# cnosdb/cnosdb

Hardware: AMD Instinct MI355X
Metric: decoded+filtered values/sec & HBM GB/s, TSBS devops scan, 1/2/4/8 GPU (higher is better)
Workload: dtype f64; 1 GPU; tsbs-devops-scan (BASELINE configs[1]: 10k series x 1M pts, reference-shaped 125k-row pages, delta-ts + Gorilla-f64 decode, ts-range filter 50%, fused 5-min max/sum/count); series_per_gpu=10000, fields=1, page_rows=125000, n_buckets=3334, raw_page_bytes_per_gpu=7320251367, sub_batches=2

## Files before the change

### cnosdb_amd/csrc/gs_engine.cpp

```cpp
#include <hip/hip_runtime.h>
#include "../../include/cnosdb_gs.h"
#include "gs_internal.h"

#pragma clang diagnostic ignored "-Wunused-value"

#include <cstdio>
#include <cstring>
#include <cstdlib>
#include <vector>
#include <algorithm>
#include <string>

static thread_local char g_err[512] = "";
static GsStatus fail(GsStatus s, const char *msg) {
    snprintf(g_err, sizeof(g_err), "%s", msg);
    return s;
}
extern "C" const char *gs_last_error(void) { return g_err; }

#define HIP_TRY(expr)                                                          \
    do {                                                                       \
        hipError_t _e = (expr);                                                \
        if (_e != hipSuccess) {                                                \
            snprintf(g_err, sizeof(g_err), "%s: %s", #expr,                    \
// ... 2313 lines not shown
    const int lane = threadIdx.x;
    int64_t carry = 0;
    for (int t = 0; t < nblocks; t += 64) {
        int i = t + lane;
        int64_t v = (i < nblocks) ? blocksums[i] : 0;
        int64_t x = v;
        for (int off = 1; off < 64; off <<= 1) {
            int64_t u = __shfl_up(x, off, 64);
            if (lane >= off) x += u;
        }
        if (i < nblocks) blocksums[i] = carry + x - v;
        carry += __shfl(x, 63, 64);
    }
    if (lane == 0) out[n] = carry;
}

__global__ void k_scan_add(int n, int64_t *__restrict__ out,
                           const int64_t *__restrict__ blocksums) {
    int chunk = SCAN_BLOCK * SCAN_ITEMS;
    for (int i = blockIdx.x * blockDim.x + threadIdx.x; i < n;
         i += gridDim.x * blockDim.x)
        out[i] += blocksums[i / chunk];
}

__global__ void k_build_sgroups_out(const int32_t *__restrict__ first,
                                    int nsg,
                                    const int64_t *__restrict__ out_off,
                                    DevGroup *__restrict__ sg) {
    for (int s = blockIdx.x * blockDim.x + threadIdx.x; s < nsg;
         s += gridDim.x * blockDim.x) {
        int64_t a = out_off[first[s]];
        int64_t b = out_off[first[s + 1]];
        sg[s].row_off = a;
        sg[s].nrows = int32_t(b - a);
        sg[s].pad = 0;
    }
}

__global__ void k_spans_rle(const uint8_t *__restrict__ blob,
                            const DevPage *__restrict__ pages, int npages,
                            int64_t lo, int64_t hi,
                            int64_t *__restrict__ sp_start,
                            int64_t *__restrict__ sp_cnt,
                            int64_t *__restrict__ g_t0sel,
                            int64_t *__restrict__ g_delta,
                            unsigned *__restrict__ err) {
    for (int p = blockIdx.x * blockDim.x + threadIdx.x; p < npages;
         p += gridDim.x * blockDim.x) {
        DevPage pg = pages[p];
        const uint8_t *s = blob + pg.data_off + 1;
        uint64_t scaler = 1;
        unsigned s10 = s[0] & 0x0f;
        for (unsigned k = 0; k < s10; k++) scaler *= 10;
        const uint8_t *q = s + 1;
        int64_t first = int64_t(dev_be64(q));
        uint64_t dv; uint32_t nr;
        dev_varint(q + 8, pg.data_len - 10, &dv, &nr);
        int64_t delta = int64_t(dv * scaler);
        int64_t n = pg.nrows;
        int64_t st, en;
        if (delta < 0) { atomicOr(err, DERR_NONMONO); st = en = 0; }
        else if (delta == 0) {
            bool in = first >= lo && first <= hi;
            st = 0; en = in ? n : 0;
        } else {
            __int128 d = delta;
            __int128 a = (__int128)lo - first;
            __int128 b = (__int128)hi - first;
            __int128 s0 = a <= 0 ? 0 : (a + d - 1) / d;
            __int128 e0 = b < 0 ? 0 : b / d + 1;
            if (s0 > n) s0 = n;
            if (e0 > n) e0 = n;
            st = int64_t(s0);
            en = int64_t(e0);
        }
        if (en < st) en = st;
        sp_start[pg.grp] = st;
        sp_cnt[pg.grp] = en - st;
        g_t0sel[pg.grp] = first + st * delta;
        g_delta[pg.grp] = delta;
    }
}

__global__ void k_rle_ts_filtered(const uint8_t *__restrict__ blob,
                                  const DevPage *__restrict__ pages,
                                  int npages,
                                  const int64_t *__restrict__ sp_start,
                                  const int64_t *__restrict__ sp_cnt,
                                  const int64_t *__restrict__ out_off,
                                  int64_t *__restrict__ out_ts) {
    for (int p = blockIdx.x; p < npages; p += gridDim.x) {
        DevPage pg = pages[p];
        const uint8_t *s = blob + pg.data_off + 1;
        uint64_t scaler = 1;
        unsigned s10 = s[0] & 0x0f;
        for (unsigned k = 0; k < s10; k++) scaler *= 10;
        const uint8_t *q = s + 1;
        int64_t first = int64_t(dev_be64(q));
        uint64_t dv; uint32_t nr;
        dev_varint(q + 8, pg.data_len - 10, &dv, &nr);
        int64_t delta = int64_t(dv * scaler);
        int64_t st = sp_start[pg.grp], cnt = sp_cnt[pg.grp];
        int64_t *o = out_ts + out_off[pg.grp];
        const uint64_t base = uint64_t(first) + uint64_t(st) * uint64_t(delta);
        const int64_t head = int64_t((uintptr_t(o) >> 3) & 1);
        if (head && threadIdx.x == 0 && cnt > 0) o[0] = int64_t(base);
        const int64_t n2 = (cnt - head) >> 1;
        longlong2 *op = (longlong2 *)(o + head);
        for (int64_t q2 = threadIdx.x; q2 < n2; q2 += blockDim.x) {
            const uint64_t r0 = uint64_t(head) + 2 * uint64_t(q2);
            longlong2 v;
            v.x = int64_t(base + r0 * uint64_t(delta));
            v.y = int64_t(base + (r0 + 1) * uint64_t(delta));
            op[q2] = v;
        }
        if (((cnt - head) & 1) && threadIdx.x == 0 && cnt > 0)
            o[cnt - 1] = int64_t(base + uint64_t(cnt - 1) * uint64_t(delta));
    }
}

__global__ void k_gor_active(const DevGorChunk *__restrict__ chunks,
                             int nchunks,
                             const int64_t *__restrict__ sp_start,
                             const int64_t *__restrict__ sp_cnt,
                             int *__restrict__ active,
                             int *__restrict__ n_active,
                             DevAggMeta *__restrict__ pieces) {
    const int lane = threadIdx.x & 63;
    for (int i = blockIdx.x * blockDim.x + threadIdx.x; i < nchunks;
         i += gridDim.x * blockDim.x) {
        uint32_t grp = chunks[i].grp;
        int64_t row0 = int64_t(chunks[i].row0);
        int64_t rend = row0 + int64_t(chunks[i].cnt);
        int64_t lo = sp_start[grp];
        int64_t hi = lo + sp_cnt[grp];
        bool act = row0 < hi && rend > lo;
        if (pieces && !act) {
            uint32_t slot = chunks[i].slot;
            if (slot != GOR_NO_SLOT)
                *(int4 *)(pieces + 2 * size_t(slot)) =
                    make_int4(AGG_NO_PIECE, 0, AGG_NO_PIECE, 0);
        }
        uint64_t m = __ballot(act);
        if (m) {
            int leader = __ffsll((unsigned long long)m) - 1;
            int base = 0;
            if (lane == leader) base = atomicAdd(n_active, __popcll(m));
            base = __shfl(base, leader);
            if (act)
                active[base + __popcll(m & ((1ull << lane) - 1))] = i;
        }
    }
}

struct GorAggArgs {
    const int32_t *grp_sg;
    const int64_t *g_t0sel;
    const int64_t *g_delta;
    int64_t t0, bucket_ns;
    int nbuckets;
    double *pmax, *psum;
    long long *pcnt;
    DevAggMeta *pc_meta;
    DevAggVal *pc_val;
};

#define GS_AGG_FUSED_MIN_ROWS 2

#define GOR_PARK_NB (1 << 30)
#define GOR_FK_END 0
#define GOR_FK_CLEAN 1
#define GOR_FK_OVER 2

template <bool AGG>
__global__ void k_gor_chunks_filtered(const uint8_t *__restrict__ blob,
                                      const DevGorChunk *__restrict__ chunks,
                                      const int *__restrict__ active,
                                      const int *__restrict__ n_active,
                                      const int64_t *__restrict__ sp_start,
                                      const int64_t *__restrict__ sp_cnt,
                                      const int64_t *__restrict__ out_off,
                                      double *__restrict__ out,
                                      unsigned *__restrict__ err,
                                      GorAggArgs ag) {
    __shared__ double ring[GS_GOR_BLOCK / 64][GS_RING][64 + 1];
    __shared__ uint64_t fdesc[GS_GOR_BLOCK / 64][64][2];
    const int lane = threadIdx.x & 63;
    const int wv = threadIdx.x >> 6;
    auto rslot = ring[wv];
    const int nact = *n_active;
    int stride = gridDim.x * blockDim.x;
    int base_id = blockIdx.x * blockDim.x + threadIdx.x;
    int rounds = (nact + stride - 1) / stride;
    for (int rd = 0; rd < rounds; rd++) {
        int ai = base_id + rd * stride;
        bool have = ai < nact;
        DevGorChunk ch = chunks[active[have ? ai : 0]];
        int32_t sel_lo = int32_t(sp_start[ch.grp]);
        int32_t sel_hi = int32_t(sel_lo + sp_cnt[ch.grp]);
        if (!have) { sel_lo = 0; sel_hi = 0; }
// ... 535 lines not shown
    __syncthreads();
    for (int p = blockIdx.x * blockDim.x + threadIdx.x; p < npages;
         p += gridDim.x * blockDim.x) {
        EncPageSpec ps = pages[p];
        uint8_t *pg = out + int64_t(p) * cap;
        uint32_t bl = uint32_t(ps.nrows + 7) / 8;
        uint8_t *bs = pg + 16;
        for (uint32_t b = 0; b < bl; b++) {
            uint8_t byte = 0;
            for (int k = 0; k < 8; k++) {
                int32_t r = int32_t(b) * 8 + k;
                if (r < ps.nrows && (!valid || valid[ps.row_off + r]))
                    byte |= uint8_t(1u << k);
            }
            bs[b] = byte;
        }
        uint8_t *data = pg + 16 + bl;
        int64_t dl;
        if (kind == 2) {
            dl = dev_enc_gorilla((const double *)vals, valid, ps.row_off,
                                 ps.nrows, data);
        } else {
            if (valid) {
                bool av = true;
                for (int32_t r = 0; r < ps.nrows; r++)
                    if (!valid[ps.row_off + r]) { av = false; break; }
                if (!av) { atomicOr(err, DERR_FORMAT); lens[p] = -3; continue; }
            }
            dl = dev_enc_int((const int64_t *)vals, ps.row_off, ps.nrows,
                             data, kind == 0);
        }
        if (dl < 0) {
            atomicOr(err, DERR_FORMAT);
            lens[p] = dl;
            continue;
        }
        uint32_t crc = 0xFFFFFFFFu;
        for (int64_t i = 0; i < dl; i++)
            crc = crct[(crc ^ data[i]) & 0xFF] ^ (crc >> 8);
        crc ^= 0xFFFFFFFFu;
        pg[0] = uint8_t(bl >> 24); pg[1] = uint8_t(bl >> 16);
        pg[2] = uint8_t(bl >> 8); pg[3] = uint8_t(bl);
        dev_put_be64(pg + 4, uint64_t(ps.nrows));
        pg[12] = uint8_t(crc >> 24); pg[13] = uint8_t(crc >> 16);
        pg[14] = uint8_t(crc >> 8); pg[15] = uint8_t(crc);
        lens[p] = 16 + int64_t(bl) + dl;
    }
}


struct GsCtx {
    int device;
    hipStream_t stream;
    unsigned *d_err;
};

static int grid_for(int work, int per_block) {
    int blocks = (work + per_block - 1) / per_block;
    if (blocks > 2048) blocks = 2048;
    if (blocks < 1) blocks = 1;
    return blocks;
}

struct SlotPages {
    uint8_t ctype;
    std::vector<DevPage> host[PC_NCLASS];
    DevPage *dev[PC_NCLASS] = {nullptr, nullptr, nullptr};
    int n[PC_NCLASS] = {0, 0, 0};
    std::vector<int64_t> str_scr;
    int64_t str_total = 0;
    int64_t *d_str_scr = nullptr;
    DevGorChunk *d_gor_chunks = nullptr;
    int n_gor_chunks = 0;
    int32_t *d_gor_chunk_base = nullptr;
    DevGorChunk *d_gorn_chunks = nullptr;
    int n_gorn_chunks = 0;
    int32_t *d_gorn_chunk_base = nullptr;
    std::vector<int32_t> gor_grp_cbase;
    int32_t *d_sg_chunk_first = nullptr;
    int max_sg_chunks = 0;
    bool agg_fused_ok = false;
};

struct GsGroupSet {
    GsCtx *ctx = nullptr;
    uint8_t *d_blob = nullptr;
    size_t blob_len = 0;
    int64_t total_rows = 0;
    size_t ngroups = 0;
    uint32_t ncols = 0;
    std::vector<int64_t> row_offsets;
    std::vector<SlotPages> slots;
    DevGroup *d_groups = nullptr;
    DevGroup *d_sgroups = nullptr;
    int nsgroups = 0;
    std::vector<int32_t> sgroup_span;
    std::vector<int64_t> sgroup_row_off;
    DevGroup *d_sgroups_out = nullptr;
    int32_t *d_sgroup_first = nullptr;
    int64_t *d_blocksums = nullptr;
    hipEvent_t sev[6];
    bool sev_init = false;
    bool pending = false;
    int64_t *d_sp_start = nullptr;
    int64_t *d_sp_cnt = nullptr;
    int64_t *d_out_off = nullptr;
    int64_t *d_g_t0sel = nullptr;
    int64_t *d_g_delta = nullptr;
    int max_span = 0;
    int *d_gor_active = nullptr;
    int *d_gor_nactive = nullptr;
    size_t gor_active_cap = 0;
    int32_t *d_grp_sgroup = nullptr;
    DevAggMeta *d_agg_meta = nullptr;
    DevAggVal *d_agg_val = nullptr;
    size_t agg_pieces_cap = 0;
    int64_t min_pos_delta = INT64_MAX;
    uint8_t *d_str_scratch = nullptr;
    size_t str_scratch_cap = 0;
    int64_t *d_str_sz = nullptr;
    int64_t *d_str_pos = nullptr;
    int64_t *d_str_bsums = nullptr;
    size_t str_bsums_cap = 0;
    GsTimeRange *d_ranges = nullptr;
    size_t ranges_cap = 0;
    uint8_t *d_valid = nullptr;
    uint8_t *d_mask = nullptr;
    int64_t *d_sel_cnt = nullptr;
    bool any_nulls_field = false;
    double *d_pmax = nullptr;
    double *d_psum = nullptr;
    long long *d_pcnt = nullptr;
    size_t partials_cap = 0;
};

extern "C" {

int gs_device_count(void) {
    int n = 0;
    if (hipGetDeviceCount(&n) != hipSuccess) return 0;
    return n;
}

GsCtx *gs_ctx_create(int device) {
    int n = 0;
    if (hipGetDeviceCount(&n) != hipSuccess || n == 0) {
        fail(GS_ERR_NO_GPU, "no HIP device available — cnosdb_gs has no CPU fallback");
        return nullptr;
    }
    if (device < 0 || device >= n) {
        fail(GS_ERR, "device index out of range");
        return nullptr;
    }
    HIP_TRY_NULL(hipSetDevice(device));
    GsCtx *ctx = new GsCtx();
    ctx->device = device;
    if (hipStreamCreate(&ctx->stream) != hipSuccess ||
        hipMalloc(&ctx->d_err, sizeof(unsigned)) != hipSuccess) {
        fail(GS_ERR, "ctx init failed");
        delete ctx;
        return nullptr;
    }
    hipMemset(ctx->d_err, 0, sizeof(unsigned));
    return ctx;
}

void gs_ctx_destroy(GsCtx *ctx) {
    if (!ctx) return;
    hipSetDevice(ctx->device);
    hipStreamSynchronize(ctx->stream);
    hipFree(ctx->d_err);
    hipStreamDestroy(ctx->stream);
    delete ctx;
}

GsGroupSet *gs_groups_upload(GsCtx *ctx, const GsColumnGroupDesc *groups,
                             size_t ngroups, int validate_crc) {
    if (!ctx || !groups || ngroups == 0) {
        fail(GS_ERR, "bad args to gs_groups_upload");
        return nullptr;
    }
    HIP_TRY_NULL(hipSetDevice(ctx->device));
    uint32_t ncols = groups[0].npages;
    for (size_t g = 0; g < ngroups; g++) {
// ... 391 lines not shown
        hipMalloc(&set->d_sgroup_first, sgfirst.size() * sizeof(int32_t)) != hipSuccess ||
        hipMalloc(&set->d_sgroups_out, hsg.size() * sizeof(DevGroup)) != hipSuccess ||
        hipMalloc(&set->d_g_t0sel, ngroups * sizeof(int64_t)) != hipSuccess ||
        hipMalloc(&set->d_g_delta, ngroups * sizeof(int64_t)) != hipSuccess) {
        fail(GS_ERR, "hipMalloc group tables failed");
        gs_groups_free(set); return nullptr;
    }
    for (int32_t sp : set->sgroup_span)
        if (sp > set->max_span) set->max_span = sp;
    hipMemcpyAsync(set->d_sgroup_first, sgfirst.data(),
                   sgfirst.size() * sizeof(int32_t), hipMemcpyHostToDevice,
                   ctx->stream);
    hipMemcpyAsync(set->d_groups, hg.data(), ngroups * sizeof(DevGroup),
                   hipMemcpyHostToDevice, ctx->stream);
    std::vector<int32_t> grp_sg(ngroups);
    for (size_t s = 0; s < hsg.size(); s++)
        for (int32_t g = sgfirst[s]; g < sgfirst[s + 1]; g++)
            grp_sg[g] = int32_t(s);
    std::vector<std::vector<int32_t>> sgc(ncols);
    if (hipMalloc(&set->d_grp_sgroup, ngroups * sizeof(int32_t)) != hipSuccess) {
        fail(GS_ERR, "hipMalloc group->sgroup table failed");
        gs_groups_free(set); return nullptr;
    }
    hipMemcpyAsync(set->d_grp_sgroup, grp_sg.data(),
                   ngroups * sizeof(int32_t), hipMemcpyHostToDevice,
                   ctx->stream);
    for (uint32_t c = 0; c < ncols; c++) {
        SlotPages &sp = set->slots[c];
        if (!sp.agg_fused_ok) continue;
        std::vector<int32_t> &t = sgc[c];
        t.resize(hsg.size() + 1);
        for (size_t s = 0; s <= hsg.size(); s++)
            t[s] = sp.gor_grp_cbase[sgfirst[s]];
        if (t[0] != 0 || t[hsg.size()] > sp.n_gor_chunks)
            sp.agg_fused_ok = false;
        for (size_t s = 0; s < hsg.size() && sp.agg_fused_ok; s++) {
            if (t[s + 1] < t[s]) sp.agg_fused_ok = false;
            if (t[s + 1] - t[s] > sp.max_sg_chunks)
                sp.max_sg_chunks = t[s + 1] - t[s];
        }
        if (!sp.agg_fused_ok) continue;
        if (hipMalloc(&sp.d_sg_chunk_first, t.size() * sizeof(int32_t)) != hipSuccess) {
            fail(GS_ERR, "hipMalloc sgroup chunk table failed");
            gs_groups_free(set); return nullptr;
        }
        hipMemcpyAsync(sp.d_sg_chunk_first, t.data(),
                       t.size() * sizeof(int32_t), hipMemcpyHostToDevice,
                       ctx->stream);
    }
    HIP_TRY_NULL(hipStreamSynchronize(ctx->stream));
    return set;
}

void gs_groups_free(GsGroupSet *set) {
    if (!set) return;
    hipSetDevice(set->ctx->device);
    hipStreamSynchronize(set->ctx->stream);
    for (auto &sp : set->slots) {
        for (int k = 0; k < PC_NCLASS; k++)
            if (sp.dev[k]) hipFree(sp.dev[k]);
        if (sp.d_str_scr) hipFree(sp.d_str_scr);
        if (sp.d_gor_chunks) hipFree(sp.d_gor_chunks);
        if (sp.d_gor_chunk_base) hipFree(sp.d_gor_chunk_base);
        if (sp.d_gorn_chunks) hipFree(sp.d_gorn_chunks);
        if (sp.d_gorn_chunk_base) hipFree(sp.d_gorn_chunk_base);
        if (sp.d_sg_chunk_first) hipFree(sp.d_sg_chunk_first);
    }
    if (set->d_grp_sgroup) hipFree(set->d_grp_sgroup);
    if (set->d_agg_meta) hipFree(set->d_agg_meta);
    if (set->d_agg_val) hipFree(set->d_agg_val);
    if (set->d_gor_active) hipFree(set->d_gor_active);
    if (set->d_gor_nactive) hipFree(set->d_gor_nactive);
    if (set->d_str_scratch) hipFree(set->d_str_scratch);
    if (set->d_str_sz) hipFree(set->d_str_sz);
    if (set->d_str_pos) hipFree(set->d_str_pos);
    if (set->d_str_bsums) hipFree(set->d_str_bsums);
    hipFree(set->d_blob);
    hipFree(set->d_groups);
    if (set->d_sgroups) hipFree(set->d_sgroups);
    if (set->d_sgroups_out) hipFree(set->d_sgroups_out);
    if (set->d_sgroup_first) hipFree(set->d_sgroup_first);
    if (set->d_blocksums) hipFree(set->d_blocksums);
    if (set->sev_init)
        for (int k = 0; k < 6; k++) hipEventDestroy(set->sev[k]);
    hipFree(set->d_sp_start);
    hipFree(set->d_sp_cnt);
    hipFree(set->d_out_off);
    if (set->d_g_t0sel) hipFree(set->d_g_t0sel);
    if (set->d_g_delta) hipFree(set->d_g_delta);
    if (set->d_ranges) hipFree(set->d_ranges);
    if (set->d_valid) hipFree(set->d_valid);
    if (set->d_mask) hipFree(set->d_mask);
    if (set->d_sel_cnt) hipFree(set->d_sel_cnt);
    if (set->d_pmax) hipFree(set->d_pmax);
    if (set->d_psum) hipFree(set->d_psum);
    if (set->d_pcnt) hipFree(set->d_pcnt);
    delete set;
}

int64_t gs_debug_gorn_table(GsCtx *ctx, GsGroupSet *set, uint32_t col,
                            DevGorChunk *out, int64_t cap) {
    if (!ctx || !set || col >= set->ncols) return -1;
    SlotPages &sp = set->slots[col];
    int64_t n = sp.n_gorn_chunks;
    if (!out || cap < n) return n;
    hipSetDevice(ctx->device);
    hipStreamSynchronize(ctx->stream);
    if (hipMemcpy(out, sp.d_gorn_chunks, size_t(n) * sizeof(DevGorChunk),
                  hipMemcpyDeviceToHost) != hipSuccess)
        return -1;
    return n;
}

int64_t gs_debug_read_blob(GsCtx *ctx, GsGroupSet *set, uint64_t off,
                           uint64_t len, uint8_t *out) {
    if (!ctx || !set || off + len > set->blob_len) return -1;
    hipSetDevice(ctx->device);
    hipStreamSynchronize(ctx->stream);
    if (hipMemcpy(out, set->d_blob + off, len, hipMemcpyDeviceToHost) !=
        hipSuccess)
        return -1;
    return int64_t(len);
}

int64_t gs_debug_rerun_gorn_sync(GsCtx *ctx, GsGroupSet *set,
                                 uint32_t col) {
    if (!ctx || !set || col >= set->ncols) return -1;
    SlotPages &sp = set->slots[col];
    if (!sp.n[PC_GORN]) return 0;
    hipSetDevice(ctx->device);
    const char *e = getenv("GS_GOR_CHUNK");
    long v = e ? atol(e) : 0;
    uint32_t chunk_rows = uint32_t(v >= 64 ? v : GOR_CHUNK);
    hipLaunchKernelGGL(k_gor_sync_null, dim3(grid_for(sp.n[PC_GORN], 256)),
                       dim3(256), 0, ctx->stream, set->d_blob,
                       sp.dev[PC_GORN], sp.n[PC_GORN], sp.d_gorn_chunk_base,
                       sp.d_gorn_chunks, chunk_rows);
    hipStreamSynchronize(ctx->stream);
    return 1;
}

__global__ void k_debug_crc(const uint8_t *__restrict__ p, uint64_t len,
                            uint64_t *__restrict__ out) {
    uint64_t acc = 0;
    for (uint64_t i = blockIdx.x * blockDim.x + threadIdx.x; i < len;
         i += uint64_t(gridDim.x) * blockDim.x)
        acc += (uint64_t(p[i]) + 1) * (i + 0x9e3779b97f4a7c15ULL);
    atomicAdd((unsigned long long *)out, (unsigned long long)acc);
}

int64_t gs_debug_kernel_crc(GsCtx *ctx, GsGroupSet *set, uint64_t off,
                            uint64_t len, uint64_t *out_sum) {
    if (!ctx || !set || off + len > set->blob_len) return -1;
    hipSetDevice(ctx->device);
    uint64_t *d;
    if (hipMalloc(&d, 8) != hipSuccess) return -1;
    hipMemset(d, 0, 8);
    hipLaunchKernelGGL(k_debug_crc, dim3(64), dim3(256), 0, ctx->stream,
                       set->d_blob + off, len, d);
    hipStreamSynchronize(ctx->stream);
    hipMemcpy(out_sum, d, 8, hipMemcpyDeviceToHost);
    hipFree(d);
    return 0;
}

int64_t gs_set_rows(const GsGroupSet *set) { return set ? set->total_rows : -1; }
int64_t gs_set_series(const GsGroupSet *set) { return set ? set->nsgroups : -1; }
// ... 317 lines not shown
                      (SCAN_BLOCK * SCAN_ITEMS));
    if (set->str_bsums_cap < size_t(nblocks) + 1) {
        if (set->d_str_bsums) hipFree(set->d_str_bsums);
        if (hipMalloc(&set->d_str_bsums, (size_t(nblocks) + 1) * 8) != hipSuccess)
            return fail(GS_ERR, "hipMalloc string scan sums failed");
        set->str_bsums_cap = size_t(nblocks) + 1;
    }
    hipLaunchKernelGGL(k_str_decode, dim3(grid_for(n, 256)), dim3(256), 0,
                       ctx->stream, set->d_blob, sp.dev[PC_STR], n,
                       sp.d_str_scr, set->d_str_scratch, set->d_str_sz,
                       set->d_str_pos, d_valid, ctx->d_err);
    hipLaunchKernelGGL(k_scan_partials, dim3(nblocks), dim3(SCAN_BLOCK), 0,
                       ctx->stream, set->d_str_sz, int(set->total_rows),
                       d_offsets, set->d_str_bsums);
    hipLaunchKernelGGL(k_scan_fixup, dim3(1), dim3(64), 0, ctx->stream,
                       int(set->total_rows), d_offsets, set->d_str_bsums,
                       nblocks);
    hipLaunchKernelGGL(k_scan_add, dim3(grid_for(int(set->total_rows), 256)),
                       dim3(256), 0, ctx->stream, int(set->total_rows),
                       d_offsets, set->d_str_bsums);
    int64_t total = 0;
    HIP_TRY(hipMemcpyAsync(&total, d_offsets + set->total_rows, 8,
                           hipMemcpyDeviceToHost, ctx->stream));
    HIP_TRY(hipStreamSynchronize(ctx->stream));
    GsStatus st = check_dev_err(ctx);
    if (st != GS_OK) return st;
    if (total > bytes_cap)
        return fail(GS_ERR, "string bytes buffer too small");
    hipLaunchKernelGGL(k_str_gather, dim3(grid_for(int(set->total_rows), 256)),
                       dim3(256), 0, ctx->stream, set->d_str_scratch,
                       set->d_str_pos, set->d_str_sz, d_offsets,
                       set->total_rows, d_bytes);
    HIP_TRY(hipStreamSynchronize(ctx->stream));
    *total_bytes = total;
    return check_dev_err(ctx);
}

GsStatus gs_apply_tombstone(GsCtx *ctx, GsGroupSet *set, const int64_t *d_ts,
                            uint8_t *d_valid, const GsTimeRange *ranges,
                            size_t nranges) {
    if (!ctx || !set || !d_ts || !d_valid || !ranges || nranges == 0)
        return fail(GS_ERR, "bad args to gs_apply_tombstone");
    HIP_TRY(hipSetDevice(ctx->device));
    if (set->ranges_cap < nranges) {
        if (set->d_ranges) hipFree(set->d_ranges);
        HIP_TRY(hipMalloc(&set->d_ranges, nranges * sizeof(GsTimeRange)));
        set->ranges_cap = nranges;
    }
    HIP_TRY(hipMemcpyAsync(set->d_ranges, ranges, nranges * sizeof(GsTimeRange),
                           hipMemcpyHostToDevice, ctx->stream));
    int blocks = int(set->ngroups > 2048 ? 2048 : set->ngroups);
    hipLaunchKernelGGL(k_tombstone, dim3(blocks), dim3(256), 0, ctx->stream,
                       set->d_groups, int(set->ngroups), d_ts, d_valid,
                       set->d_ranges, int(nranges));
    HIP_TRY(hipStreamSynchronize(ctx->stream));
    return GS_OK;
}

static bool fused_capable_fields(GsGroupSet *set, const GsScanSpec *spec,
                                 const int32_t *fields, int nf) {
    if (!(spec->d_out_ts && spec->d_out_val && spec->n_tombstones == 0 &&
          spec->value_pred.op == GS_PRED_NONE && !set->any_nulls_field &&
          set->slots[0].n[PC_RLE_TS] == int(set->ngroups)))
        return false;
    for (int f = 0; f < nf; f++) {
        uint32_t fc = 1 + uint32_t(fields[f]);
        if (fc >= set->ncols ||
            set->slots[fc].n[PC_GOR] != int(set->ngroups))
            return false;
    }
    return true;
}

static bool fused_capable(GsGroupSet *set, const GsScanSpec *spec) {
    int32_t f0 = spec->field_col;
    return fused_capable_fields(set, spec, &f0, 1);
}

static GsStatus scan_fused_launch(GsCtx *ctx, GsGroupSet *set,
                                  const GsScanSpec *spec,
                                  const int32_t *fields, int nf) {
    HIP_TRY(hipSetDevice(ctx->device));
    if (!set->sev_init) {
        for (int k = 0; k < 6; k++) HIP_TRY(hipEventCreate(&set->sev[k]));
        set->sev_init = true;
    }
    hipEvent_t *ev = set->sev;
    int ng = int(set->ngroups);
    const DevPage *ts_pages = set->slots[0].dev[PC_RLE_TS];
    int nch_max = 0;
    for (int f = 0; f < nf; f++) {
        int nc = set->slots[1 + fields[f]].n_gor_chunks;
        nch_max = nc > nch_max ? nc : nch_max;
    }
    if (!set->d_gor_nactive &&
        hipMalloc(&set->d_gor_nactive, sizeof(int)) != hipSuccess)
        return fail(GS_ERR, "hipMalloc active counter failed");
    if (set->gor_active_cap < size_t(nch_max)) {
        if (set->d_gor_active) hipFree(set->d_gor_active);
        if (hipMalloc(&set->d_gor_active, size_t(nch_max) * sizeof(int)) !=
            hipSuccess)
            return fail(GS_ERR, "hipMalloc active list failed");
        set->gor_active_cap = size_t(nch_max);
    }
    int nblocks = (ng + SCAN_BLOCK * SCAN_ITEMS - 1) /
                  (SCAN_BLOCK * SCAN_ITEMS);
    if (nblocks > 2048)
        return fail(GS_ERR, "too many groups for the fused span scan");
    HIP_TRY(hipEventRecord(ev[0], ctx->stream));
    hipLaunchKernelGGL(k_spans_rle, dim3(grid_for(ng, 256)), dim3(256), 0,
                       ctx->stream, set->d_blob, ts_pages, ng,
                       spec->range.min_ts, spec->range.max_ts,
                       set->d_sp_start, set->d_sp_cnt, set->d_g_t0sel,
                       set->d_g_delta, ctx->d_err);
    hipLaunchKernelGGL(k_scan_partials, dim3(nblocks), dim3(SCAN_BLOCK), 0,
                       ctx->stream, set->d_sp_cnt, ng, set->d_out_off,
                       set->d_blocksums);
    hipLaunchKernelGGL(k_scan_fixup, dim3(1), dim3(64), 0, ctx->stream, ng,
                       set->d_out_off, set->d_blocksums, nblocks);
    hipLaunchKernelGGL(k_scan_add, dim3(grid_for(ng, 256)), dim3(256), 0,
                       ctx->stream, ng, set->d_out_off, set->d_blocksums);
    HIP_TRY(hipEventRecord(ev[1], ctx->stream));
    hipLaunchKernelGGL(k_rle_ts_filtered, dim3(ng > 2048 ? 2048 : ng),
                       dim3(256), 0, ctx->stream, set->d_blob, ts_pages, ng,
                       set->d_sp_start, set->d_sp_cnt, set->d_out_off,
                       spec->d_out_ts);
    HIP_TRY(hipEventRecord(ev[2], ctx->stream));
    int nsg = set->nsgroups;
    if (spec->n_buckets > 0) {
        if (!spec->d_agg_max || !spec->d_agg_sum || !spec->d_agg_count)
            return fail(GS_ERR, "agg outputs missing");
        size_t cells = size_t(nsg) * size_t(spec->n_buckets);
        if (set->partials_cap < cells) {
            if (set->d_pmax) hipFree(set->d_pmax);
            if (set->d_psum) hipFree(set->d_psum);
            if (set->d_pcnt) hipFree(set->d_pcnt);
            if (hipMalloc(&set->d_pmax, cells * 8) != hipSuccess ||
                hipMalloc(&set->d_psum, cells * 8) != hipSuccess ||
                hipMalloc(&set->d_pcnt, cells * 8) != hipSuccess)
                return fail(GS_ERR, "hipMalloc agg partials failed");
            set->partials_cap = cells;
        }
    }
    bool sgroups_built = false;
    auto build_sgroups = [&]() {
        if (sgroups_built) return;
        hipLaunchKernelGGL(k_build_sgroups_out, dim3(grid_for(nsg, 256)),
                           dim3(256), 0, ctx->stream, set->d_sgroup_first,
                           nsg, set->d_out_off, set->d_sgroups_out);
        sgroups_built = true;
    };
    for (int f = 0; f < nf; f++) {
        SlotPages &fsp = set->slots[1 + fields[f]];
        int nch = fsp.n_gor_chunks;
        double *d_val_f = spec->d_out_val + size_t(f) * set->total_rows;
        HIP_TRY(hipMemsetAsync(set->d_gor_nactive, 0, sizeof(int),
                               ctx->stream));
        const size_t shm_rle =
            size_t(set->max_span) * 16 +
            (size_t(set->max_span) + size_t(spec->n_buckets) + 2) * 4;
        const bool rle_fits =
            spec->n_buckets <= 8192 && shm_rle <= 64 * 1024;
        const size_t shm_fix =
            (size_t(fsp.max_sg_chunks) * 2 * 4 + size_t(spec->n_buckets) +
             15) & ~size_t(15);
        bool agg_fused = false;
        if (spec->n_buckets > 0 && rle_fits && fsp.agg_fused_ok &&
            spec->bucket_ns > 0 && shm_fix <= 64 * 1024) {
            static int fused_env = [] {
                const char *e = getenv("GS_AGG_FUSED");
                return e ? atoi(e) : 1;
            }();
            static long min_rows = [] {
                const char *e = getenv("GS_AGG_FUSED_MIN_ROWS");
                long v = e ? atol(e) : 0;
                return v > 0 ? v : long(GS_AGG_FUSED_MIN_ROWS);
            }();
            agg_fused = fused_env != 0 &&
                        (set->min_pos_delta == INT64_MAX ||
                         spec->bucket_ns / set->min_pos_delta >= min_rows);
        }
        if (agg_fused && set->agg_pieces_cap < size_t(nch_max) * 2) {
            if (set->d_agg_meta) hipFree(set->d_agg_meta);
            if (set->d_agg_val) hipFree(set->d_agg_val);
            set->d_agg_meta = nullptr;
            set->d_agg_val = nullptr;
            set->agg_pieces_cap = 0;
            if (hipMalloc(&set->d_agg_meta, size_t(nch_max) * 2 *
                                                sizeof(DevAggMeta)) !=
                    hipSuccess ||
                hipMalloc(&set->d_agg_val, size_t(nch_max) * 2 *
                                               sizeof(DevAggVal)) !=
                    hipSuccess)
                return fail(GS_ERR, "hipMalloc agg pieces failed");
            set->agg_pieces_cap = size_t(nch_max) * 2;
        }
        hipLaunchKernelGGL(k_gor_active, dim3(grid_for(nch, 256)), dim3(256),
                           0, ctx->stream, fsp.d_gor_chunks, nch,
                           set->d_sp_start, set->d_sp_cnt, set->d_gor_active,
                           set->d_gor_nactive,
                           agg_fused ? set->d_agg_meta : nullptr);
        GorAggArgs ag{};
        if (agg_fused) {
            ag.grp_sg = set->d_grp_sgroup;
            ag.g_t0sel = set->d_g_t0sel;
            ag.g_delta = set->d_g_delta;
            ag.t0 = spec->t0;
            ag.bucket_ns = spec->bucket_ns;
            ag.nbuckets = spec->n_buckets;
            ag.pmax = set->d_pmax;
            ag.psum = set->d_psum;
            ag.pcnt = set->d_pcnt;
            ag.pc_meta = set->d_agg_meta;
            ag.pc_val = set->d_agg_val;
            hipLaunchKernelGGL(k_gor_chunks_filtered<true>,
                               dim3(grid_for(nch, GS_GOR_BLOCK)),
                               dim3(GS_GOR_BLOCK), 0, ctx->stream,
                               set->d_blob, fsp.d_gor_chunks,
                               set->d_gor_active, set->d_gor_nactive,
                               set->d_sp_start, set->d_sp_cnt,
                               set->d_out_off, d_val_f, ctx->d_err, ag);
        } else {
            hipLaunchKernelGGL(k_gor_chunks_filtered<false>,
                               dim3(grid_for(nch, GS_GOR_BLOCK)),
                               dim3(GS_GOR_BLOCK), 0, ctx->stream,
                               set->d_blob, fsp.d_gor_chunks,
                               set->d_gor_active, set->d_gor_nactive,
                               set->d_sp_start, set->d_sp_cnt,
                               set->d_out_off, d_val_f, ctx->d_err, ag);
        }
        if (f == 0) HIP_TRY(hipEventRecord(ev[3], ctx->stream));
        if (spec->n_buckets > 0) {
            if (agg_fused) {
                hipLaunchKernelGGL(k_agg_fixup,
                                   dim3(nsg > 65535 ? 65535 : nsg),
                                   dim3(256), shm_fix, ctx->stream,
                                   set->d_agg_meta, set->d_agg_val,
                                   fsp.d_sg_chunk_first,
                                   nsg, spec->n_buckets,
                                   fsp.max_sg_chunks * 2, set->d_pmax,
                                   set->d_psum, set->d_pcnt);
            } else if (rle_fits) {
                static int agg_block = [] {
                    const char *e = getenv("GS_AGG_BLOCK");
                    long v = e ? atol(e) : 0;
                    return int(v == 128 || v == 512 ? v : 256);
                }();
                build_sgroups();
                hipLaunchKernelGGL(k_agg_partial_rle,
                                   dim3(nsg > 65535 ? 65535 : nsg),
                                   dim3(agg_block), shm_rle, ctx->stream,
                                   set->d_sgroups_out, nsg,
                                   set->d_sgroup_first, set->d_g_t0sel,
                                   set->d_g_delta, set->d_out_off, d_val_f,
                                   spec->t0, spec->bucket_ns,
                                   spec->n_buckets, set->max_span,
                                   set->d_pmax, set->d_psum, set->d_pcnt);
            } else {
                size_t agg_shm = spec->n_buckets <= 8192
                                     ? (size_t(spec->n_buckets) + 1) * 4
                                     : 0;
                build_sgroups();
                hipLaunchKernelGGL(
                    k_agg_partial, dim3(nsg > 65535 ? 65535 : nsg),
                    dim3(256), agg_shm, ctx->stream, set->d_sgroups_out,
                    nsg, spec->d_out_ts, d_val_f, nullptr, INT64_MIN,
                    INT64_MAX, spec->t0, spec->bucket_ns, spec->n_buckets,
                    set->d_pmax, set->d_psum, set->d_pcnt);
            }
            int mb = (spec->n_buckets + 3) / 4;
            hipLaunchKernelGGL(k_agg_merge, dim3(mb > 2048 ? 2048 : mb),
                               dim3(256), 0, ctx->stream, nsg,
                               spec->n_buckets, set->d_pmax, set->d_psum,
                               set->d_pcnt,
                               spec->d_agg_max + size_t(f) * spec->n_buckets,
                               spec->d_agg_sum + size_t(f) * spec->n_buckets,
                               spec->d_agg_count +
                                   size_t(f) * spec->n_buckets);
        }
    }
    HIP_TRY(hipEventRecord(ev[4], ctx->stream));
    HIP_TRY(hipEventRecord(ev[5], ctx->stream));
    set->pending = true;
    return GS_OK;
}

static GsStatus scan_fused_wait(GsCtx *ctx, GsGroupSet *set,
                                GsScanResult *result) {
    if (!set->pending)
        return fail(GS_ERR, "no fused scan in flight on this set");
    set->pending = false;
    HIP_TRY(hipStreamSynchronize(ctx->stream));
    GsStatus st = check_dev_err(ctx);
    if (st != GS_OK) return st;
    int64_t acc = 0;
    HIP_TRY(hipMemcpy(&acc, set->d_out_off + set->ngroups, sizeof(int64_t),
                      hipMemcpyDeviceToHost));
    hipEvent_t *ev = set->sev;
    float ms;
    HIP_TRY(hipEventElapsedTime(&ms, ev[0], ev[1]));
    result->ms_filter = ms;
    HIP_TRY(hipEventElapsedTime(&ms, ev[1], ev[2]));
    result->ms_decode_ts = ms;
    HIP_TRY(hipEventElapsedTime(&ms, ev[2], ev[3]));
    result->ms_decode_val = ms;
    result->ms_compact = 0.0;
    HIP_TRY(hipEventElapsedTime(&ms, ev[3], ev[4]));
    result->ms_agg = ms;
    result->out_rows = acc;
    result->decoded_rows = set->total_rows;
    return GS_OK;
}

GsStatus gs_scan_async(GsCtx *ctx, GsGroupSet *set, const GsScanSpec *spec) {
    if (!ctx || !set || !spec)
        return fail(GS_ERR, "bad args to gs_scan_async");
    if (!fused_capable(set, spec))
        return fail(GS_ERR, "gs_scan_async requires the fused-capable shape "
                            "(RLE ts + all-valid Gorilla, no tombstones, "
                            "compacted outputs)");
    int32_t f0 = spec->field_col;
    return scan_fused_launch(ctx, set, spec, &f0, 1);
}

GsStatus gs_scan_wait(GsCtx *ctx, GsGroupSet *set, GsScanResult *result) {
    if (!ctx || !set || !result)
        return fail(GS_ERR, "bad args to gs_scan_wait");
    return scan_fused_wait(ctx, set, result);
}

GsGroupSet *gs_raw_set(GsCtx *ctx, const int64_t *counts, int64_t nseries) {
    if (!ctx || !counts || nseries <= 0) {
        fail(GS_ERR, "bad args to gs_raw_set");
        return nullptr;
    }
    if (hipSetDevice(ctx->device) != hipSuccess) {
        fail(GS_ERR, "hipSetDevice failed");
        return nullptr;
    }
    GsGroupSet *set = new GsGroupSet();
    set->ctx = ctx;
    set->ngroups = size_t(nseries);
    set->ncols = 0;
    set->row_offsets.resize(nseries);
    std::vector<DevGroup> hg(nseries);
    int64_t rows = 0;
    for (int64_t i = 0; i < nseries; i++) {
        if (counts[i] < 0 || counts[i] > INT32_MAX) {
            fail(GS_ERR, "raw set series row count out of range");
            gs_groups_free(set);
            return nullptr;
        }
        set->row_offsets[i] = rows;
        hg[i].row_off = rows;
        hg[i].nrows = int32_t(counts[i]);
        hg[i].pad = 0;
        rows += counts[i];
    }
    set->total_rows = rows;
    set->nsgroups = int(nseries);
    set->sgroup_span.assign(nseries, 1);
    set->max_span = 1;
    std::vector<int32_t> sgfirst(nseries + 1);
    for (int64_t i = 0; i <= nseries; i++) sgfirst[i] = int32_t(i);
    size_t nblocks = (size_t(nseries) + SCAN_BLOCK * SCAN_ITEMS - 1) /
                     (SCAN_BLOCK * SCAN_ITEMS);
    if (hipMalloc(&set->d_groups, nseries * sizeof(DevGroup)) != hipSuccess ||
        hipMalloc(&set->d_sgroups, nseries * sizeof(DevGroup)) != hipSuccess ||
        hipMalloc(&set->d_sgroups_out, nseries * sizeof(DevGroup)) != hipSuccess ||
        hipMalloc(&set->d_sgroup_first, sgfirst.size() * sizeof(int32_t)) != hipSuccess ||
        hipMalloc(&set->d_sp_start, nseries * sizeof(int64_t)) != hipSuccess ||
        hipMalloc(&set->d_sp_cnt, nseries * sizeof(int64_t)) != hipSuccess ||
        hipMalloc(&set->d_out_off, (nseries + 1) * sizeof(int64_t)) != hipSuccess ||
        hipMalloc(&set->d_blocksums, (nblocks + 1) * sizeof(int64_t)) != hipSuccess) {
        fail(GS_ERR, "hipMalloc raw set tables failed");
        gs_groups_free(set);
        return nullptr;
    }
    hipMemcpyAsync(set->d_groups, hg.data(), nseries * sizeof(DevGroup),
                   hipMemcpyHostToDevice, ctx->stream);
    hipMemcpyAsync(set->d_sgroups, hg.data(), nseries * sizeof(DevGroup),
                   hipMemcpyHostToDevice, ctx->stream);
    hipMemcpyAsync(set->d_sgroup_first, sgfirst.data(),
                   sgfirst.size() * sizeof(int32_t), hipMemcpyHostToDevice,
                   ctx->stream);
    if (hipStreamSynchronize(ctx->stream) != hipSuccess) {
        fail(GS_ERR, "raw set upload failed");
        gs_groups_free(set);
        return nullptr;
    }
// ... 517 lines not shown
```

Measured before the change: 315.3 billion values/s.

## Write filtered RLE timestamps in fixed row tiles instead of per-page blocks

Replaces the per-page timestamp kernel with a tile-based kernel. Each block takes a fixed range of output rows and finds the owning groups by binary search over out_off. It reads the precomputed t0sel and delta instead of re-parsing page headers, and steps each value by addition instead of multiplying. This balances work across blocks when selected counts vary between groups, at the cost of a search per tile and of requiring g_t0sel/g_delta to be filled. The event array is also reduced from six entries to five with named indices.

```diff
diff --git a/cnosdb_amd/csrc/gs_engine.cpp b/cnosdb_amd/csrc/gs_engine.cpp
--- a/cnosdb_amd/csrc/gs_engine.cpp
+++ b/cnosdb_amd/csrc/gs_engine.cpp
@@ -2419,40 +2419,59 @@
     }
 }
 
-__global__ void k_rle_ts_filtered(const uint8_t *__restrict__ blob,
-                                  const DevPage *__restrict__ pages,
-                                  int npages,
-                                  const int64_t *__restrict__ sp_start,
-                                  const int64_t *__restrict__ sp_cnt,
-                                  const int64_t *__restrict__ out_off,
-                                  int64_t *__restrict__ out_ts) {
-    for (int p = blockIdx.x; p < npages; p += gridDim.x) {
-        DevPage pg = pages[p];
-        const uint8_t *s = blob + pg.data_off + 1;
-        uint64_t scaler = 1;
-        unsigned s10 = s[0] & 0x0f;
-        for (unsigned k = 0; k < s10; k++) scaler *= 10;
-        const uint8_t *q = s + 1;
-        int64_t first = int64_t(dev_be64(q));
-        uint64_t dv; uint32_t nr;
-        dev_varint(q + 8, pg.data_len - 10, &dv, &nr);
-        int64_t delta = int64_t(dv * scaler);
-        int64_t st = sp_start[pg.grp], cnt = sp_cnt[pg.grp];
-        int64_t *o = out_ts + out_off[pg.grp];
-        const uint64_t base = uint64_t(first) + uint64_t(st) * uint64_t(delta);
-        const int64_t head = int64_t((uintptr_t(o) >> 3) & 1);
-        if (head && threadIdx.x == 0 && cnt > 0) o[0] = int64_t(base);
-        const int64_t n2 = (cnt - head) >> 1;
-        longlong2 *op = (longlong2 *)(o + head);
-        for (int64_t q2 = threadIdx.x; q2 < n2; q2 += blockDim.x) {
-            const uint64_t r0 = uint64_t(head) + 2 * uint64_t(q2);
-            longlong2 v;
-            v.x = int64_t(base + r0 * uint64_t(delta));
-            v.y = int64_t(base + (r0 + 1) * uint64_t(delta));
-            op[q2] = v;
-        }
-        if (((cnt - head) & 1) && threadIdx.x == 0 && cnt > 0)
-            o[cnt - 1] = int64_t(base + uint64_t(cnt - 1) * uint64_t(delta));
+#define GS_TS_TILE 16384
+
+__device__ __forceinline__ int ts_group_of(const int64_t *__restrict__ out_off,
+                                           int g0, int ngroups, int64_t r) {
+    int lo = g0, hi = ngroups - 1;
+    while (lo < hi) {
+        int mid = lo + ((hi - lo) >> 1);
+        if (out_off[mid + 1] > r) hi = mid;
+        else lo = mid + 1;
+    }
+    return lo;
+}
+
+__global__ __launch_bounds__(256) void k_rle_ts_tiles(
+    const int64_t *__restrict__ out_off, int ngroups,
+    const int64_t *__restrict__ g_t0sel, const int64_t *__restrict__ g_delta,
+    int tile, int64_t *__restrict__ out_ts) {
+    const int64_t first = out_off[0];
+    const int64_t total = out_off[ngroups];
+    const int64_t ntiles = (total - first + tile - 1) / tile;
+    for (int64_t t = blockIdx.x; t < ntiles; t += gridDim.x) {
+        int64_t r = first + t * tile;
+        const int64_t r_end = r + tile < total ? r + tile : total;
+        int g = ts_group_of(out_off, 0, ngroups, r);
+        while (true) {
+            const int64_t g_first = out_off[g], g_end = out_off[g + 1];
+            const int64_t seg_end = g_end < r_end ? g_end : r_end;
+            const int64_t cnt = seg_end - r;
+            const uint64_t delta = uint64_t(g_delta[g]);
+            const uint64_t base =
+                uint64_t(g_t0sel[g]) + uint64_t(r - g_first) * delta;
+            int64_t *o = out_ts + r;
+            const int64_t head = int64_t((uintptr_t(o) >> 3) & 1);
+            if (head && threadIdx.x == 0) o[0] = int64_t(base);
+            const int64_t n2 = (cnt - head) >> 1;
+            longlong2 *op = (longlong2 *)(o + head);
+            uint64_t v0 =
+                base + (uint64_t(head) + 2 * uint64_t(threadIdx.x)) * delta;
+            const uint64_t step = 2 * uint64_t(blockDim.x) * delta;
+            for (int64_t q2 = threadIdx.x; q2 < n2; q2 += blockDim.x) {
+                longlong2 v;
+                v.x = int64_t(v0);
+                v.y = int64_t(v0 + delta);
+                op[q2] = v;
+                v0 += step;
+            }
+            if (((cnt - head) & 1) && threadIdx.x == 0)
+                o[cnt - 1] = int64_t(base + uint64_t(cnt - 1) * delta);
+            r = seg_end;
+            if (r >= r_end) break;
+            g = out_off[g + 2] > r ? g + 1
+                                   : ts_group_of(out_off, g + 2, ngroups, r);
+        }
     }
 }
 
@@ -3154,6 +3173,8 @@
     bool agg_fused_ok = false;
 };
 
+enum { SEV_START, SEV_OFFS, SEV_TS, SEV_VAL, SEV_END, GS_NSEV };
+
 struct GsGroupSet {
     GsCtx *ctx = nullptr;
     uint8_t *d_blob = nullptr;
@@ -3171,7 +3192,7 @@
     DevGroup *d_sgroups_out = nullptr;
     int32_t *d_sgroup_first = nullptr;
     int64_t *d_blocksums = nullptr;
-    hipEvent_t sev[6];
+    hipEvent_t sev[GS_NSEV];
     bool sev_init = false;
     bool pending = false;
     int64_t *d_sp_start = nullptr;
@@ -3729,7 +3750,7 @@
     if (set->d_sgroup_first) hipFree(set->d_sgroup_first);
     if (set->d_blocksums) hipFree(set->d_blocksums);
     if (set->sev_init)
-        for (int k = 0; k < 6; k++) hipEventDestroy(set->sev[k]);
+        for (int k = 0; k < GS_NSEV; k++) hipEventDestroy(set->sev[k]);
     hipFree(set->d_sp_start);
     hipFree(set->d_sp_cnt);
     hipFree(set->d_out_off);
@@ -4213,7 +4234,8 @@
                                   const int32_t *fields, int nf) {
     HIP_TRY(hipSetDevice(ctx->device));
     if (!set->sev_init) {
-        for (int k = 0; k < 6; k++) HIP_TRY(hipEventCreate(&set->sev[k]));
+        for (int k = 0; k < GS_NSEV; k++)
+            HIP_TRY(hipEventCreate(&set->sev[k]));
         set->sev_init = true;
     }
     hipEvent_t *ev = set->sev;
@@ -4238,7 +4260,7 @@
                   (SCAN_BLOCK * SCAN_ITEMS);
     if (nblocks > 2048)
         return fail(GS_ERR, "too many groups for the fused span scan");
-    HIP_TRY(hipEventRecord(ev[0], ctx->stream));
+    HIP_TRY(hipEventRecord(ev[SEV_START], ctx->stream));
     hipLaunchKernelGGL(k_spans_rle, dim3(grid_for(ng, 256)), dim3(256), 0,
                        ctx->stream, set->d_blob, ts_pages, ng,
                        spec->range.min_ts, spec->range.max_ts,
@@ -4251,12 +4273,13 @@
                        set->d_out_off, set->d_blocksums, nblocks);
     hipLaunchKernelGGL(k_scan_add, dim3(grid_for(ng, 256)), dim3(256), 0,
                        ctx->stream, ng, set->d_out_off, set->d_blocksums);
-    HIP_TRY(hipEventRecord(ev[1], ctx->stream));
-    hipLaunchKernelGGL(k_rle_ts_filtered, dim3(ng > 2048 ? 2048 : ng),
-                       dim3(256), 0, ctx->stream, set->d_blob, ts_pages, ng,
-                       set->d_sp_start, set->d_sp_cnt, set->d_out_off,
-                       spec->d_out_ts);
-    HIP_TRY(hipEventRecord(ev[2], ctx->stream));
+    HIP_TRY(hipEventRecord(ev[SEV_OFFS], ctx->stream));
+    int64_t tiles = (set->total_rows + GS_TS_TILE - 1) / GS_TS_TILE;
+    tiles = tiles < 1 ? 1 : (tiles > 2048 ? 2048 : tiles);
+    hipLaunchKernelGGL(k_rle_ts_tiles, dim3(int(tiles)), dim3(256), 0,
+                       ctx->stream, set->d_out_off, ng, set->d_g_t0sel,
+                       set->d_g_delta, GS_TS_TILE, spec->d_out_ts);
+    HIP_TRY(hipEventRecord(ev[SEV_TS], ctx->stream));
     int nsg = set->nsgroups;
     if (spec->n_buckets > 0) {
         if (!spec->d_agg_max || !spec->d_agg_sum || !spec->d_agg_count)
@@ -4360,7 +4383,7 @@
                                set->d_sp_start, set->d_sp_cnt,
                                set->d_out_off, d_val_f, ctx->d_err, ag);
         }
-        if (f == 0) HIP_TRY(hipEventRecord(ev[3], ctx->stream));
+        if (f == 0) HIP_TRY(hipEventRecord(ev[SEV_VAL], ctx->stream));
         if (spec->n_buckets > 0) {
             if (agg_fused) {
                 hipLaunchKernelGGL(k_agg_fixup,
@@ -4410,8 +4433,7 @@
                                    size_t(f) * spec->n_buckets);
         }
     }
-    HIP_TRY(hipEventRecord(ev[4], ctx->stream));
-    HIP_TRY(hipEventRecord(ev[5], ctx->stream));
+    HIP_TRY(hipEventRecord(ev[SEV_END], ctx->stream));
     set->pending = true;
     return GS_OK;
 }
@@ -4429,14 +4451,14 @@
                       hipMemcpyDeviceToHost));
     hipEvent_t *ev = set->sev;
     float ms;
-    HIP_TRY(hipEventElapsedTime(&ms, ev[0], ev[1]));
+    HIP_TRY(hipEventElapsedTime(&ms, ev[SEV_START], ev[SEV_OFFS]));
     result->ms_filter = ms;
-    HIP_TRY(hipEventElapsedTime(&ms, ev[1], ev[2]));
+    HIP_TRY(hipEventElapsedTime(&ms, ev[SEV_OFFS], ev[SEV_TS]));
     result->ms_decode_ts = ms;
-    HIP_TRY(hipEventElapsedTime(&ms, ev[2], ev[3]));
+    HIP_TRY(hipEventElapsedTime(&ms, ev[SEV_TS], ev[SEV_VAL]));
     result->ms_decode_val = ms;
     result->ms_compact = 0.0;
-    HIP_TRY(hipEventElapsedTime(&ms, ev[3], ev[4]));
+    HIP_TRY(hipEventElapsedTime(&ms, ev[SEV_VAL], ev[SEV_END]));
     result->ms_agg = ms;
     result->out_rows = acc;
     result->decoded_rows = set->total_rows;
```

After: 361.6 billion values/s, median of 6. +14.7%, better.
